# kyotovision-public/DRMNet

Measured on NVIDIA B200. Metric: refmaps rendered/sec (128^2, 2000x1000 envmap), higher is better.
Workload: dtype f32

## Files before the change

### drmnet_b200/csrc/render_tree.cu

```cuda
#include <cuda_fp16.h>
#include <math.h>
#include <string.h>

#include "common.cuh"

namespace drm {

static constexpr int TREE_THREADS = 256;
static constexpr int TREE_WARPS = 8;
static constexpr int REC4 = 5;
static constexpr int SREC4 = 7;
static constexpr int PAIR4 = 13;
static constexpr int MAX_PYR = 14;
static constexpr int STACK_CAP = 1024;
static constexpr int BUF1 = 32;
static constexpr int BUF0 = 32;
static constexpr int TREE_MAX_P = 4;
static constexpr int CHUNK = 128;
static constexpr int TREE_CHUNK = 64;

struct PyrGeom {
    int L, base;
    int H[MAX_PYR], W[MAX_PYR];
    long off[MAX_PYR];
// ... 153 lines not shown
        if (!(o > 0.f)) return;
        if (!any) { any = true; ref[0] = g0.x; ref[1] = g0.y; ref[2] = g0.z; }
        const float dx = g0.x - ref[0], dy = g0.y - ref[1], dz = g0.z - ref[2];
        om += o;
        s1[0] += o * dx; s1[1] += o * dy; s1[2] += o * dz;
        s2[0] += o * (g1.x + dx * dx); s2[1] += o * (g1.y + dy * dy); s2[2] += o * (g1.z + dz * dz);
        s2[3] += o * (g1.w + dx * dy); s2[4] += o * (g2.x + dx * dz); s2[5] += o * (g2.y + dy * dz);
        w[0] += g2.z; w[1] += g2.w; w[2] += g3.x;
        cR[0] += g3.y + g2.z * dx; cR[1] += g3.z + g2.z * dy; cR[2] += g3.w + g2.z * dz;
        cB[0] += g4.x + g3.x * dx; cB[1] += g4.y + g3.x * dy; cB[2] += g4.z + g3.x * dz;
    }
    __device__ __forceinline__ void finish(float4* r, float rh, float* mu_out) const {
        if (!any) {
            for (int i = 0; i < REC4; ++i) r[i] = make_float4(0.f, 0.f, 0.f, 0.f);
            mu_out[0] = mu_out[1] = mu_out[2] = 0.f;
            return;
        }
        const float io = 1.f / om;
        const float ax = s1[0] * io, ay = s1[1] * io, az = s1[2] * io;
        mu_out[0] = ref[0] + ax; mu_out[1] = ref[1] + ay; mu_out[2] = ref[2] + az;
        r[0] = make_float4(mu_out[0], mu_out[1], mu_out[2], rh);
        r[1] = make_float4(fmaxf(s2[0] * io - ax * ax, 0.f), fmaxf(s2[1] * io - ay * ay, 0.f), fmaxf(s2[2] * io - az * az, 0.f),
                           s2[3] * io - ax * ay);
        r[2] = make_float4(s2[4] * io - ax * az, s2[5] * io - ay * az, w[0], w[1]);
        r[3] = make_float4(w[2], cR[0] - w[0] * ax, cR[1] - w[0] * ay, cR[2] - w[0] * az);
        r[4] = make_float4(cB[0] - w[2] * ax, cB[1] - w[2] * ay, cB[2] - w[2] * az, 0.f);
    }
};

__device__ __forceinline__ float texel_f(float x) { return x; }
__device__ __forceinline__ float texel_f(__half x) { return __half2float(x); }

template <typename T>
__device__ __forceinline__ void texel_spec(const TreeArgs& g, const TreeConst& rc, const T* __restrict__ env_b, int r,
                                           int c, float* h, float& vh, float* w) {
    const float st = g.sin_t[r], ct = g.cos_t[r], sp = g.sin_p[c], cp = g.cos_p[c];
    const float dx = st * sp, dy = ct, dz = -st * cp;
    const float dom = g.domega_k * st;
    const T* e = env_b + ((size_t)r * g.We + c) * 3;
    const float sx = rc.vhat[0] + dx, sy = rc.vhat[1] + dy, sz = rc.vhat[2] + dz;
    const float len2 = fmaxf(sx * sx + sy * sy + sz * sz, 1e-12f);
    const float inv_len = rsqrtf(len2);
    vh = 0.5f * len2 * inv_len;
    h[0] = sx * inv_len; h[1] = sy * inv_len; h[2] = sz * inv_len;
    const float Fd = fresnel_dielectric_t(vh, rc.eta);
    const float mm = fminf(fmaxf(1.f - vh, 0.f), 1.f);
    const float sw = (mm * mm) * (mm * mm) * mm;
    const float a = (1.f - rc.m) * Fd + rc.m * sw, b = rc.m * (1.f - sw);
    w[0] = texel_f(e[0]) * dom * (a + b * rc.base[0]);
    w[1] = texel_f(e[1]) * dom * (a + b * rc.base[1]);
    w[2] = texel_f(e[2]) * dom * (a + b * rc.base[2]);
}

template <typename T>
__device__ __forceinline__ void texel_diff(const TreeArgs& g, const T* __restrict__ env_b, int r, int c, float* d,
                                           float* w) {
    const float st = g.sin_t[r], ct = g.cos_t[r], sp = g.sin_p[c], cp = g.cos_p[c];
    d[0] = st * sp; d[1] = ct; d[2] = -st * cp;
    const float dom = g.domega_k * st;
    const T* e = env_b + ((size_t)r * g.We + c) * 3;
    w[0] = texel_f(e[0]) * dom; w[1] = texel_f(e[1]) * dom; w[2] = texel_f(e[2]) * dom;
}

__global__ void tree_mark_used_kernel(const TreeConst* __restrict__ rc, int N, int* __restrict__ used) {
    const int k = blockIdx.x * blockDim.x + threadIdx.x;
    if (k < N && rc[k].has_diff) used[rc[k].env] = 1;
}

__global__ void env_mark_slots_kernel(const int32_t* __restrict__ ids, int n, int B, int* __restrict__ used) {
    const int i = blockIdx.x * blockDim.x + threadIdx.x;
    if (!ids) {
        if (i < B) used[i] = 1;
    } else if (i < n) {
        const int e = ids[i];
        if (e >= 0 && e < B) used[e] = 1;
    }
}

__global__ void tree_active_kernel(const TreeConst* __restrict__ rc, int n, int* __restrict__ act, int* __restrict__ nact) {
    if (blockIdx.x != 0 || threadIdx.x != 0) return;
    for (int p = 0; p <= TREE_MAX_P; ++p) {
        int c = 0;
        for (int k = 0; k < n; ++k)
            if (rc[k].pk >= p) act[p * TREE_CHUNK + c++] = k;
        nact[p] = c;
    }
}

template <bool SPEC, typename T>
__device__ __forceinline__ void pyr_from_texels(const TreeArgs& g, int lev, float4* __restrict__ pyr) {
    const PyrGeom& G = SPEC ? g.gs : g.gd;
    const int Hl = G.H[lev], Wl = G.W[lev];
    const int cell = blockIdx.x * blockDim.x + threadIdx.x;
    if (cell >= Hl * Wl) return;
    const int k = blockIdx.y;
    if (!SPEC && !g.env_used[k]) return;
    const int R = cell / Wl, C = cell - R * Wl;
    const int e = 1 << lev;
    const TreeConst* rcp = SPEC ? &g.rc[k] : nullptr;
    const T* env_b = reinterpret_cast<const T*>(g.env) + (size_t)(SPEC ? rcp->env : k) * g.He * g.We * 3;
    float4* rec = pyr + ((size_t)k * G.cells + G.off[lev] + cell) * REC4;
    if (SPEC && !rcp->has_spec) {
        for (int i = 0; i < REC4; ++i) rec[i] = make_float4(0.f, 0.f, 0.f, 0.f);
        return;
    }
    Mom M;
    M.init();
    const int r1 = min((R + 1) * e, g.He), c1 = min((C + 1) * e, g.We);
    for (int r = R * e; r < r1; ++r)
        for (int c = C * e; c < c1; ++c) {
            float x[3], w[3], vh;
            if (SPEC) texel_spec(g, *rcp, env_b, r, c, x, vh, w);
            else texel_diff(g, env_b, r, c, x, w);
            M.add_point(x, w);
        }
    float4 out[REC4];
    float mu[3];
    M.finish(out, 0.f, mu);
    float rh = 0.f;
    if (M.any) {
        for (int r = R * e; r < r1; ++r)
            for (int c = C * e; c < c1; ++c) {
                float x[3], w[3], vh;
                if (SPEC) texel_spec(g, *rcp, env_b, r, c, x, vh, w);
                else texel_diff(g, env_b, r, c, x, w);
                if (w[0] + w[1] + w[2] > 0.f) {
                    const float dx = x[0] - mu[0], dy = x[1] - mu[1], dz = x[2] - mu[2];
                    rh = fmaxf(rh, dx * dx + dy * dy + dz * dz);
                }
            }
        out[0].w = sqrtf(rh) * 1.0001f + 1e-7f;
    }
    for (int i = 0; i < REC4; ++i) rec[i] = out[i];
}

template <bool SPEC>
__global__ void pyr_from_texels_kernel(const TreeArgs g, int lev, float4* __restrict__ pyr) {
    pyr_from_texels<SPEC, float>(g, lev, pyr);
}
template <bool SPEC>
__global__ void pyr_from_texels_kernel_h(const TreeArgs g, int lev, float4* __restrict__ pyr) {
    pyr_from_texels<SPEC, __half>(g, lev, pyr);
}

__global__ void pyr_merge_kernel(PyrGeom G, int lev, float4* __restrict__ pyr, const int* __restrict__ used) {
    const int Hl = G.H[lev], Wl = G.W[lev], Hc = G.H[lev - 1], Wc = G.W[lev - 1];
    const int cell = blockIdx.x * blockDim.x + threadIdx.x;
    if (cell >= Hl * Wl) return;
    if (used && !used[blockIdx.y]) return;
    const int R = cell / Wl, C = cell - R * Wl;
    float4* base = pyr + (size_t)blockIdx.y * G.cells * REC4;
    const float4* child = base + G.off[lev - 1] * REC4;
    Mom M;
    M.init();
    for (int dr = 0; dr < 2; ++dr)
        for (int dc = 0; dc < 2; ++dc) {
            const int r = 2 * R + dr, c = 2 * C + dc;
            if (r < Hc && c < Wc) M.add_record(child + ((size_t)r * Wc + c) * REC4);
        }
    float4 out[REC4];
    float mu[3];
    M.finish(out, 0.f, mu);
    if (M.any) {
        float rh = 0.f;
        for (int dr = 0; dr < 2; ++dr)
            for (int dc = 0; dc < 2; ++dc) {
                const int r = 2 * R + dr, c = 2 * C + dc;
                if (r >= Hc || c >= Wc) continue;
                const float4* ch = child + ((size_t)r * Wc + c) * REC4;
                const float4 g0 = ch[0], g2 = ch[2], g3 = ch[3];
                if (!(g2.z + g2.w + g3.x > 0.f)) continue;
                const float dx = g0.x - mu[0], dy = g0.y - mu[1], dz = g0.z - mu[2];
                rh = fmaxf(rh, sqrtf(dx * dx + dy * dy + dz * dz) + g0.w);
            }
        out[0].w = rh * 1.0001f + 1e-7f;
    }
    float4* rec = base + (G.off[lev] + cell) * REC4;
    for (int i = 0; i < REC4; ++i) rec[i] = out[i];
}

__device__ __forceinline__ float view_term_t(const TreeConst& rc, float lz) {
    const float g1 = lz + sqrtf(lz * lz * rc.one_m_a2 + rc.alpha2);
    return lz > 0.f ? 1.f / (3.14159265358979f * rc.alpha2 * g1) : 0.f;
}

struct NodeT {
    float nx, ny, nz, nv, mult, wq, Fi;
    float q0, q1, q2, q3, q4, q5;
    float P0, P1, P2, P3, P4, P5;
    bool active;
};

__device__ __forceinline__ void make_node(const TreeArgs& g, const TreeConst& rc, int p, bool pixcov, int I, int J, bool spec,
                                          NodeT& nd) {
    const int pk = rc.pk, Sk = 1 << p, S = 1 << pk;
    const float* __restrict__ glx = g.glx[p];
// ... 92 lines not shown
}

enum : int { ACT_DROP = 0, ACT_ACCEPT = 1, ACT_REFINE = 2, ACT_HAND = 3 };

typedef float2 f2;
__device__ __forceinline__ f2 F2(float a) { return make_float2(a, a); }
__device__ __forceinline__ f2 fma2(f2 a, f2 b, f2 c) { return __ffma2_rn(a, b, c); }
__device__ __forceinline__ f2 mul2(f2 a, f2 b) { return __fmul2_rn(a, b); }
__device__ __forceinline__ f2 add2(f2 a, f2 b) { return __fadd2_rn(a, b); }
__device__ __forceinline__ f2 sub2(f2 a, f2 b) { return __fadd2_rn(a, make_float2(-b.x, -b.y)); }
__device__ __forceinline__ f2 max2(f2 a, float s) { return make_float2(fmaxf(a.x, s), fmaxf(a.y, s)); }
__device__ __forceinline__ f2 rcp2(f2 a) { return make_float2(fast_rcp(a.x), fast_rcp(a.y)); }
__device__ __forceinline__ f2 rsqrt2(f2 a) { return make_float2(fast_rsqrt(a.x), fast_rsqrt(a.y)); }
__device__ __forceinline__ f2 sqrt2(f2 a) { return make_float2(fast_sqrt(a.x), fast_sqrt(a.y)); }
__device__ __forceinline__ f2 lo(float4 v) { return make_float2(v.x, v.y); }
__device__ __forceinline__ f2 hi(float4 v) { return make_float2(v.z, v.w); }

__device__ __forceinline__ void tile_writeback(const TreeArgs& g, int p, float* red, int k, int ti, int tj, float a0, float a1,
                                               float a2, bool overwrite) {
    const int tid = threadIdx.x, lane = tid & 31, warp = tid >> 5;
    const int ln = ((warp >> 1) * 4 + (lane >> 3)) * 16 + (warp & 1) * 8 + (lane & 7);
    red[ln * 3 + 0] = a0; red[ln * 3 + 1] = a1; red[ln * 3 + 2] = a2;
    __syncthreads();
    const int Sk = 1 << p, cpt = 16 >> p;
    if (cpt < 1) return;
    const int ncell = cpt * cpt;
    for (int o = tid; o < ncell * 3; o += TREE_THREADS) {
        const int cl = o / 3, c = o - cl * 3;
        const int ci = cl / cpt, cj = cl - ci * cpt;
        const int i = ti * cpt + ci, j = tj * cpt + cj;
        if (i >= g.res || j >= g.res) continue;
        float v = 0.f;
        for (int a = 0; a < Sk; ++a)
            for (int b = 0; b < Sk; ++b) v += red[((ci * Sk + a) * 16 + cj * Sk + b) * 3 + c];
        const size_t pix = (size_t)i * g.res + j;
        const size_t idx = g.channel_first ? ((size_t)k * 3 + c) * g.res * g.res + pix : ((size_t)k * g.res * g.res + pix) * 3 + c;
        g.out[idx] = overwrite ? v : g.out[idx] + v;
    }
}

__device__ __forceinline__ void tile_of(int t, int tiles_x, int& ti, int& tj) {
    const int m = tiles_x - 1;
    if (tiles_x <= 2) { ti = t / tiles_x; tj = t - ti * tiles_x; }
    else if (t < tiles_x) { ti = 0; tj = t; }
    else if (t < 2 * tiles_x) { ti = m; tj = t - tiles_x; }
    else if (t < 2 * tiles_x + (m - 1)) { ti = 1 + t - 2 * tiles_x; tj = 0; }
    else if (t < 4 * m) { ti = 1 + t - 2 * tiles_x - (m - 1); tj = m; }
    else { const int q = t - 4 * m; ti = 1 + q / (m - 1); tj = 1 + q - (ti - 1) * (m - 1); }
}

static constexpr int SPEC_MINB[TREE_MAX_P + 1] = {3, 3, 3, 3, 3}, DIFF_MINB = 3;

static constexpr int STAT_TILE_WAIT = 50, STAT_WARP_CYCLES = 56;

struct WarpUni {
    float ax, ay, az, beta;
    float thr_p, hand_p, hz_p, xthr, rcap, kappa2;
    int limb;
};

template <int P, typename T>
__device__ __forceinline__ void tree_spec_pass(const TreeArgs g, int tid) {
    extern __shared__ __align__(16) unsigned char tree_smem[];
    const int lane = tid & 31, warp = tid >> 5;
    int* stack = reinterpret_cast<int*>(tree_smem) + warp * STACK_CAP;
    float* buf1 = reinterpret_cast<float*>(tree_smem + TREE_WARPS * STACK_CAP * 4) + warp * (BUF1 / 2 * PAIR4 * 4);
    float4* buf0 = reinterpret_cast<float4*>(tree_smem + TREE_WARPS * STACK_CAP * 4 + TREE_WARPS * (BUF1 / 2) * PAIR4 * 16) + warp * (BUF0 * 2);
    float* red = reinterpret_cast<float*>(tree_smem);

    constexpr int p = P;
    const int NG = g.res << p;
    const int tiles_x = (NG + 15) / 16;
    const int n_items = g.nact[p] * tiles_x * tiles_x;
    const bool stats = g.stats;
    long long t_warp = stats ? clock64() : 0, t_wait = 0;
    auto tile_sync = [&]() {
        const long long t = stats ? clock64() : 0;
        __syncthreads();
        if (stats) t_wait += clock64() - t;
    };
    __shared__ int next_item, next_k;
    __shared__ TreeConst rc;
    __shared__ WarpUni wu_s[TREE_WARPS];
    WarpUni& wu = wu_s[warp];
    while (true) {
    if (warp == 0) {
        int it = 0;
        if (lane == 0) it = atomicAdd(g.item_ctr, 1);
        it = __shfl_sync(0xffffffffu, it, 0);
        if (it < n_items) {
            const int kk = g.act[p * TREE_CHUNK + it % g.nact[p]];
            const int* src = reinterpret_cast<const int*>(g.rc + kk);
            int* dst = reinterpret_cast<int*>(&rc);
            for (int i = lane; i < (int)(sizeof(TreeConst) / 4); i += 32) dst[i] = src[i];
            if (lane == 0) next_k = kk;
        }
        if (lane == 0) next_item = it;
    }
    tile_sync();
    const int item = next_item;
    if (item >= n_items) break;
    const int k = next_k;
    const int tile = item / g.nact[p];
    const int pk = rc.pk;
    int ti, tj;
    tile_of(tile, tiles_x, ti, tj);
    const int I0 = ti * 16 + (warp >> 1) * 4, J0 = tj * 16 + (warp & 1) * 8;
    float a0 = 0.f, a1 = 0.f, a2 = 0.f;
    const bool pixcov = g.pixcov && p == 0 && pk > 0;

    NodeT nd;
    make_node(g, rc, p, pixcov, I0 + (lane >> 3), J0 + (lane & 7), true, nd);
    float ax, ay, az, beta;
    const bool live = rc.has_spec && warp_cone(g, p, nd, ax, ay, az, beta);
// ... 170 lines not shown
                float* s = reinterpret_cast<float*>(buf0 + (n0 >> 1) * 4) + 1;
                if (lane < 7) s[lane * 2] = lane < 3 ? (lane == 0 ? nd.nx : lane == 1 ? nd.ny : nd.nz) : 0.f;
                __syncwarp();
            }
            const int np = (n0 + 1) >> 1;
            f2 bR = F2(0.f), bG = F2(0.f), bB = F2(0.f);
#pragma unroll 2
            for (int j = 0; j < np; ++j) {
                const float4 v0 = buf0[4 * j], v1 = buf0[4 * j + 1], v2 = buf0[4 * j + 2], v3 = buf0[4 * j + 3];
                const f2 ex = sub2(NX, lo(v0)), ey = sub2(NY, hi(v0)), ez = sub2(NZ, lo(v1));
                const f2 u2 = fma2(ez, ez, fma2(ey, ey, mul2(ex, ex)));
                const f2 nh = fma2(u2, F2(-0.5f), F2(1.f));
                const f2 xc = max2(sub2(mul2(hi(v1), nh), NVp), 0.f);
                const f2 sin2 = mul2(u2, fma2(u2, F2(-0.25f), F2(1.f)));
                const f2 q = fma2(sin2, CI, F2(1.f));
                const f2 sq = sqrt2(fma2(mul2(xc, xc), OMA, A2));
                const f2 ws = mul2(xc, rcp2(mul2(mul2(q, q), add2(xc, sq))));
                bR = fma2(ws, lo(v2), bR); bG = fma2(ws, hi(v2), bG); bB = fma2(ws, lo(v3), bB);
            }
            a0 += nd.mult * (bR.x + bR.y); a1 += nd.mult * (bG.x + bG.y); a2 += nd.mult * (bB.x + bB.y);
            n0 = 0;
        };

        bool done = false;
        while (true) {
            unsigned ent = 0;
            int ntake;
            if (sp > 0) {
                ntake = min(32, sp);
                if (lane < ntake) ent = (unsigned)stack[sp - 1 - lane];
                sp -= ntake;
            } else {
                if (p > 0 && in_pos >= in_n && in_next >= 0) {
                    const int* ch = g.pool_in + (size_t)in_next * CHUNK;
                    in_next = ch[0];
                    in_n = ch[1];
                    in_list = ch + 2;
                    in_pos = 0;
                }
                if (in_pos < in_n) {
                    ntake = min(32, in_n - in_pos);
                    if (lane < ntake) ent = p == 0 ? (((unsigned)g.gs.L << 28) | (unsigned)(in_pos + lane)) : (unsigned)in_list[in_pos + lane];
                    in_pos += ntake;
                } else {
                    ntake = 0;
                    done = true;
                }
            }
            const bool has = lane < ntake;
            st_visits += ntake; st_iters += 1;
            __syncwarp();
            int act = ACT_DROP;
            const int lev = (int)(ent >> 28), id = (int)(ent & 0x0fffffffu);
            float h[3], vh = 0.f, w3[3];
            if (has) {
                float mx, my, mz, rha, wsum, vmu, im;
                if (lev > 0) {
                    const float4* rp = pyr + (g.gs.off[lev] + id) * REC4;
                    const float4 r0 = rp[0], r2 = rp[2], r3 = rp[3];
                    mx = r0.x; my = r0.y; mz = r0.z;
                    wsum = r2.z + r2.w + r3.x;
                    const float m2 = fmaxf(mx * mx + my * my + mz * mz, 1e-30f);
                    im = fast_rsqrt(m2);
                    rha = fast_radius_angle(r0.w + fmaxf(1.f - m2 * im, 0.f));
                    vmu = rc.vhat[0] * mx + rc.vhat[1] * my + rc.vhat[2] * mz;
                } else {
                    const int r = id / g.We, c = id - r * g.We;
                    texel_spec(g, rc, env_b, r, c, h, vh, w3);
                    mx = h[0]; my = h[1]; mz = h[2];
                    wsum = w3[0] + w3[1] + w3[2];
                    im = 1.f; rha = 0.f; vmu = vh;
                }
                if (wsum > 0.f) {
                    const float ax = wu.ax, ay = wu.ay, az = wu.az, beta = wu.beta;
                    const float hx = mx * im - ax, hy = my * im - ay, hz = mz * im - az;
                    const float ang = fast_chord_angle(hx * hx + hy * hy + hz * hz);
                    const float dmin = fmaxf(ang - beta - rha, 0.f);
                    const float t2 = 2.f * vmu * im * im;
                    const float adc = ax * (t2 * mx - rc.vhat[0]) + ay * (t2 * my - rc.vhat[1]) + az * (t2 * mz - rc.vhat[2]);
                    const float spread = beta + 2.f * rha + 1e-3f;
                    const float ss = __sinf(fminf(spread, 1.5607f));
                    if (spread < 1.5607f && adc <= -ss) act = ACT_DROP;
                    else if (p < pk && dmin < wu.thr_p) act = (lev == 0 || rha <= wu.hand_p * wu.thr_p) ? ACT_HAND : ACT_REFINE;
                    else if (p < pk && wu.limb && spread < 1.5607f &&
                             adc * __cosf(spread) - sqrtf(fmaxf(1.f - adc * adc, 0.f)) * ss < wu.xthr)
                        act = (lev == 0 || rha <= 0.05f) ? ACT_HAND : ACT_REFINE;
                    else if (lev > 0 && (rha > wu.rcap || rha * rha > wu.kappa2 * (rc.alpha2 + dmin * dmin) ||
                                         (2.f * rha > wu.hz_p && fabsf(adc) < ss))) act = ACT_REFINE;
                    else act = ACT_ACCEPT;
                }
            }
            {
                const unsigned mh = __ballot_sync(0xffffffffu, act == ACT_HAND);
                if (mh) {
                    const int cnt = __popc(mh);
                    if (out_cur < 0 || out_fill + cnt > CHUNK - 2) {
                        int nc = 0;
                        if (lane == 0) nc = atomicAdd(g.pool_ctr, 1);
                        nc = __shfl_sync(0xffffffffu, nc, 0);
                        if (nc >= g.pool_cap) {
                            if (lane == 0) atomicOr(g.status, 1);
                            nc = -1;
                        }
                        if (lane == 0) {
                            if (out_cur >= 0) {
                                g.pool_out[(size_t)out_cur * CHUNK] = nc;
                                g.pool_out[(size_t)out_cur * CHUNK + 1] = out_fill;
                            }
                        }
                        if (out_cur < 0) out_head = nc;
                        out_cur = nc;
                        out_fill = 0;
                    }
                    if (act == ACT_HAND && out_cur >= 0)
                        g.pool_out[(size_t)out_cur * CHUNK + 2 + out_fill + __popc(mh & ((1u << lane) - 1u))] = (int)ent;
                    if (out_cur >= 0) out_fill += cnt;
                    out_n += cnt;
                }
// ... 53 lines not shown
                        s[8] = Sxx; s[10] = Syy; s[12] = Szz; s[14] = 2.f * Sxy; s[16] = 2.f * Sxz; s[18] = 2.f * Syz;
                        s[20] = 2.f * vmu / fmaxf(1.f - trS, 1e-12f);
                        s[22] = r2.z; s[24] = r2.w; s[26] = r3.x;
                        s[28] = r3.y; s[30] = r3.z; s[32] = r3.w;
                        s[34] = r4.x; s[36] = r4.y; s[38] = r4.z;
                        s[40] = vmu; s[42] = vx * svx + vy * svy + vz * svz;
                        s[44] = svx; s[46] = svy; s[48] = svz; s[50] = 0.f;
                    } else {
                        const int slot = n0 + __popc(m0 & ((1u << lane) - 1u));
                        float* s = reinterpret_cast<float*>(buf0 + (slot >> 1) * 4) + (slot & 1);
                        s[0] = h[0]; s[2] = h[1]; s[4] = h[2]; s[6] = 2.f * vh;
                        s[8] = w3[0]; s[10] = w3[1]; s[12] = w3[2];
                    }
                }
                n1 += __popc(m1);
                n0 += __popc(m0);
                st_acc1 += __popc(m1); st_acc0 += __popc(m0);
            }
            __syncwarp();
        }
        if (p < pk && lane == 0) {
            const int nbI = (NG + 3) / 4;
            if (out_cur >= 0) {
                g.pool_out[(size_t)out_cur * CHUNK] = -1;
                g.pool_out[(size_t)out_cur * CHUNK + 1] = out_fill;
            }
            g.heads_out[(size_t)k * nbI * nbJ + (size_t)bI * nbJ + bJ] = out_head;
        }
        if (lane == 0 && g.stats) {
            atomicAdd(g.status + 16 + 4 * p, st_visits); atomicAdd(g.status + 17 + 4 * p, st_iters);
            atomicAdd(g.status + 18 + 4 * p, st_acc0); atomicAdd(g.status + 19 + 4 * p, st_acc1);
        }
        if (lane == 0) {
            if (sp_max > g.status[1]) atomicMax(g.status + 1, sp_max);
            if (out_n > g.status[2 + p]) atomicMax(g.status + 2 + p, out_n);
        }
    } else if (p < pk && lane == 0) {
        const int nbJ = (NG + 7) / 8, nbI = (NG + 3) / 4;
        const int bI = I0 >> 2, bJ = J0 >> 3;
        if (bI < nbI && bJ < nbJ) g.heads_out[(size_t)k * nbI * nbJ + (size_t)bI * nbJ + bJ] = -1;
    }
    tile_sync();
    tile_writeback(g, p, red, k, ti, tj, a0, a1, a2, false);
    tile_sync();
    }
    if (stats && lane == 0) {
        atomicAdd(g.status + STAT_TILE_WAIT + p, (int)(t_wait >> 10));
        atomicAdd(g.status + STAT_WARP_CYCLES + p, (int)((clock64() - t_warp) >> 10));
    }
}

template <int P>
__global__ void __launch_bounds__(TREE_THREADS, SPEC_MINB[P]) tree_spec_pass_kernel(const TreeArgs g) {
    tree_spec_pass<P, float>(g, threadIdx.x);
}
template <int P>
__global__ void __launch_bounds__(TREE_THREADS, SPEC_MINB[P]) tree_spec_pass_kernel_h(const TreeArgs g) {
    tree_spec_pass<P, __half>(g, threadIdx.x);
}

template <typename T>
__device__ __forceinline__ void tree_diff(const TreeArgs& g, int tid) {
    extern __shared__ __align__(16) unsigned char tree_smem[];
    const int lane = tid & 31, warp = tid >> 5;
    int* stack = reinterpret_cast<int*>(tree_smem) + warp * STACK_CAP;
    float4* buf1 = reinterpret_cast<float4*>(tree_smem + TREE_WARPS * STACK_CAP * 4) + warp * (BUF1 * SREC4);
    float* red = reinterpret_cast<float*>(tree_smem);

    const int k = blockIdx.y;
    const TreeConst rc = g.rc[k];
    const int p = g.diff_cov ? 0 : rc.pk;
    const bool pixcov = g.diff_cov && rc.pk > 0;
    const int tiles_x = ((g.res << p) + 15) / 16;
    if ((int)blockIdx.x >= tiles_x * tiles_x) return;
    const int ti = blockIdx.x / tiles_x, tj = blockIdx.x - ti * tiles_x;
    const int I0 = ti * 16 + (warp >> 1) * 4, J0 = tj * 16 + (warp & 1) * 8;
    float a0 = 0.f, a1 = 0.f, a2 = 0.f;
    NodeT nd;
    make_node(g, rc, p, pixcov, I0 + (lane >> 3), J0 + (lane & 7), false, nd);
    float ax, ay, az, beta;
    const bool live = rc.has_diff && warp_cone(g, p, nd, ax, ay, az, beta);
    if (live) {
        const float4* pyr = g.pyr_d + (size_t)rc.env * g.gd.cells * REC4;
        const T* env_b = reinterpret_cast<const T*>(g.env) + (size_t)rc.env * g.He * g.We * 3;
        const int in_n = g.gd.H[g.gd.L] * g.gd.W[g.gd.L];
        int in_pos = 0, sp = 0, n1 = 0;
        const float vx = rc.vhat[0], vy = rc.vhat[1], vz = rc.vhat[2];
        const float Fi = nd.Fi, r = rc.rough;
        const float A = 1.f - 0.5f * Fi, Bc = r * Fi, Cc = -0.5f * (1.f - 0.5f * Fi), Dc = r * (1.f - Fi), Ec = r * r * Fi;
        auto eval = [&]() {
            for (int i = 0; i < n1; ++i) {
                const float4* s = buf1 + i * SREC4;
                const float4 s0 = s[0], s1 = s[1], s2 = s[2], s3 = s[3], s4 = s[4], s5 = s[5], s6 = s[6];
                float x = nd.nx * s0.x + nd.ny * s0.y + nd.nz * s0.z;
                float nSn = nd.q0 * s1.x + nd.q1 * s1.y + nd.q2 * s1.z + nd.q3 * s2.x + nd.q4 * s2.y + nd.q5 * s2.z;
                if (pixcov)
                    nSn += s0.x * s0.x * nd.P0 + s0.y * s0.y * nd.P1 + s0.z * s0.z * nd.P2 + s0.x * s0.y * nd.P3 +
                           s0.x * s0.z * nd.P4 + s0.y * s0.z * nd.P5;
                const float w = fast_sqrt(3.f * fmaxf(nSn, 0.f));
                const bool straddle = x < w;
                const float xe = fmaxf(x + w, 0.f);
                x = straddle ? (w > 0.f ? xe * xe * fast_rcp(4.f * w) : 0.f) : x;
                x = fmaxf(x, 0.f);
                const float y = s0.w;
                const float mm = fmaxf(1.f - x, 0.f);
                const float m2 = mm * mm, m4 = m2 * m2, Fo = m4 * mm;
                const float gq = Cc + y * (Dc + Ec * y);
                const float lin = A + Bc * y + Fo * gq;
                const float gy = Dc + 2.f * Ec * y;
                const float Fo1 = -5.f * m4, Fo2 = 20.f * m2 * mm;
                const float Kx = lin + x * Fo1 * gq;
// ... 143 lines not shown
    G.cells = off > 0 ? off : 1;
}

static void gauss_legendre_t(int S, float* x, float* w) {
    for (int i = 0; i < S; ++i) {
        double z = cos(M_PI * (i + 0.75) / (S + 0.5)), pp = 1.0;
        for (int it = 0; it < 100; ++it) {
            double p1 = 1.0, p2 = 0.0;
            for (int j = 0; j < S; ++j) {
                const double p3 = p2;
                p2 = p1;
                p1 = ((2.0 * j + 1.0) * z * p2 - j * p3) / (j + 1.0);
            }
            pp = S * (z * p1 - p2) / (z * z - 1.0);
            const double dz = p1 / pp;
            z -= dz;
            if (fabs(dz) < 1e-15) break;
        }
        x[S - 1 - i] = (float)z;
        w[S - 1 - i] = (float)(1.0 / ((1.0 - z * z) * pp * pp));
    }
}

struct TreeLayout {
    PyrGeom gs, gd;
    int pk;
    size_t nblocks[TREE_MAX_P];
    int pool_cap[2];
    int* status;
    int* env_used;
    int* act;
    int* nact;
    TreeConst* rc;
    float *sin_t, *cos_t, *sin_p, *cos_p;
    float4 *pyr_s, *pyr_d;
    int* pool[2];
    int* heads[2];
};

static int log2_exact(int S) {
    for (int p = 0; p <= TREE_MAX_P; ++p)
        if ((1 << p) == S) return p;
    return -1;
}

static void make_diffuse_geom(PyrGeom& G, int He, int We) {
    int dbase = 0;
    while ((2 << dbase) * M_PI / He <= 0.03) ++dbase;
    make_geom(G, He, We, dbase);
}

static size_t tree_layout(TreeLayout& L, void* ws, int N, int B, int He, int We, int res, int S, bool prepared = false) {
    make_geom(L.gs, He, We, 1);
    make_diffuse_geom(L.gd, He, We);
    L.pk = S > 0 ? log2_exact(S) : TREE_MAX_P;
    const int NC = N < TREE_CHUNK ? N : TREE_CHUNK;
    Carver c(ws);
    L.status = c.take<int>(64);
    L.rc = c.take<TreeConst>(N);
    L.env_used = prepared ? nullptr : c.take<int>(B);
    L.act = c.take<int>((TREE_MAX_P + 1) * TREE_CHUNK);
    L.nact = c.take<int>(16);
    L.sin_t = c.take<float>(He);
    L.cos_t = c.take<float>(He);
    L.sin_p = c.take<float>(We);
    L.cos_p = c.take<float>(We);
    L.pyr_s = c.take<float4>((size_t)NC * L.gs.cells * REC4);
    L.pyr_d = prepared ? nullptr : c.take<float4>((size_t)B * L.gd.cells * REC4);
    size_t need[2] = {1, 1}, needh[2] = {1, 1};
    for (int p = 0; p < L.pk; ++p) {
        const size_t NG = (size_t)res << p;
        L.nblocks[p] = ((NG + 3) / 4) * ((NG + 7) / 8);
        static const size_t budget[TREE_MAX_P] = {64, 24, 10, 6};
        const size_t per_block = budget[p];
        const size_t n = (size_t)NC * L.nblocks[p] * per_block + 64;
        if (n > need[p & 1]) need[p & 1] = n;
        if ((size_t)NC * L.nblocks[p] > needh[p & 1]) needh[p & 1] = (size_t)NC * L.nblocks[p];
    }
    for (int i = 0; i < 2; ++i) {
        L.pool_cap[i] = (int)(need[i] < 0x7fffffff / CHUNK ? need[i] : 0x7fffffff / CHUNK);
        L.pool[i] = c.take<int>((size_t)L.pool_cap[i] * CHUNK);
        L.heads[i] = c.take<int>(needh[i]);
    }
    return c.used();
}

struct EnvPyrLayout {
    PyrGeom gd;
    float4* pyr;
    float *sin_t, *cos_t, *sin_p, *cos_p;
    int* used;
};

static size_t env_pyr_layout(EnvPyrLayout& L, void* buf, int B, int He, int We) {
    make_diffuse_geom(L.gd, He, We);
    Carver c(buf);
    L.pyr = c.take<float4>((size_t)B * L.gd.cells * REC4);
    L.sin_t = c.take<float>(He);
    L.cos_t = c.take<float>(He);
    L.sin_p = c.take<float>(We);
    L.cos_p = c.take<float>(We);
    L.used = c.take<int>(B);
    return c.used();
}

static bool env_sizes_ok(int B, int He, int We) {
    return B > 0 && B <= 65535 && He > 0 && We > 0 && (long)He * We < (1L << 28);
}

static constexpr size_t TREE_SMEM = (size_t)TREE_WARPS * STACK_CAP * 4 + (size_t)TREE_WARPS * (BUF1 / 2) * PAIR4 * 16 +
                                    (size_t)TREE_WARPS * BUF0 * 2 * 16;
static_assert(BUF1 * SREC4 <= (BUF1 / 2) * PAIR4 + 8 * BUF0, "the diffuse pass stages its records in the same region");

static constexpr int MAX_DEVICES = 64;

template <typename T> struct TexelKernels;
template <> struct TexelKernels<float> {
    template <int P> static constexpr void (*spec)(TreeArgs) = tree_spec_pass_kernel<P>;
    static constexpr void (*diff)(TreeArgs) = tree_diff_kernel;
    template <bool SPEC> static constexpr void (*pyr)(TreeArgs, int, float4*) = pyr_from_texels_kernel<SPEC>;
};
template <> struct TexelKernels<__half> {
    template <int P> static constexpr void (*spec)(TreeArgs) = tree_spec_pass_kernel_h<P>;
    static constexpr void (*diff)(TreeArgs) = tree_diff_kernel_h;
    template <bool SPEC> static constexpr void (*pyr)(TreeArgs, int, float4*) = pyr_from_texels_kernel_h<SPEC>;
};

template <typename T>
static int launch_diffuse_pyramids(const TreeArgs& g, int B, float4* pyr, cudaStream_t st) {
    if (g.gd.L < 1) return 0;
    const int tb = 128;
    const int first = g.gd.base > 0 ? g.gd.base : 1;
    const int nb = g.gd.H[first] * g.gd.W[first];
    int launches = 0;
    TexelKernels<T>::template pyr<false><<<dim3((nb + tb - 1) / tb, B), tb, 0, st>>>(g, first, pyr);
    ++launches;
    for (int l = first + 1; l <= g.gd.L; ++l) {
        const int nl = g.gd.H[l] * g.gd.W[l];
        pyr_merge_kernel<<<dim3((nl + tb - 1) / tb, B), tb, 0, st>>>(g.gd, l, pyr, g.env_used);
        ++launches;
    }
    return launches;
}

template <int P, typename T>
static cudaError_t launch_spec_pass(const TreeArgs& a, long items, cudaStream_t st) {
    static int resident[MAX_DEVICES];
    void (*kernel)(TreeArgs) = TexelKernels<T>::template spec<P>;
    cudaError_t e = cudaFuncSetAttribute(kernel, cudaFuncAttributeMaxDynamicSharedMemorySize, (int)TREE_SMEM);
    if (e == cudaSuccess)
        e = cudaFuncSetAttribute(kernel, cudaFuncAttributePreferredSharedMemoryCarveout, cudaSharedmemCarveoutMaxShared);
    int dev = 0;
    if (e == cudaSuccess) e = cudaGetDevice(&dev);
    if (e != cudaSuccess) return e;
    int per_sm = 0, sms = 0;
    int* slot = dev < MAX_DEVICES ? &resident[dev] : &per_sm;
    if (*slot == 0) {
        e = cudaOccupancyMaxActiveBlocksPerMultiprocessor(&per_sm, kernel, TREE_THREADS, TREE_SMEM);
        if (e == cudaSuccess) e = cudaDeviceGetAttribute(&sms, cudaDevAttrMultiProcessorCount, dev);
        if (e != cudaSuccess) return e;
        *slot = max(per_sm, 1) * sms;
    }
    const int grid = (int)(items < *slot ? items : *slot);
    kernel<<<grid, TREE_THREADS, TREE_SMEM, st>>>(a);
    return cudaGetLastError();
}

}

using namespace drm;

extern "C" size_t drm_render_workspace_bytes(int N, int B, int He, int We, int res, int S) {
    if (N <= 0 || B <= 0 || He <= 0 || We <= 0 || res <= 0 || (S != 0 && log2_exact(S) < 0)) return 0;
    if ((long)He * We >= (1L << 28)) return 0;
    TreeLayout L;
    return tree_layout(L, nullptr, N, B, He, We, res, S);
}

extern "C" size_t drm_render_prepared_workspace_bytes(int N, int B, int He, int We, int res, int S) {
    if (N <= 0 || B <= 0 || He <= 0 || We <= 0 || res <= 0 || (S != 0 && log2_exact(S) < 0)) return 0;
    if ((long)He * We >= (1L << 28)) return 0;
    TreeLayout L;
    return tree_layout(L, nullptr, N, B, He, We, res, S, true);
}

extern "C" size_t drm_env_pyramid_bytes(int B, int He, int We) {
    if (!env_sizes_ok(B, He, We)) return 0;
    EnvPyrLayout P;
    return env_pyr_layout(P, nullptr, B, He, We);
}

template <typename T>
static int env_pyramid_build(const T* env, int B, int He, int We, const int32_t* ids, int n_ids, void* pyramids,
                             size_t pyramid_bytes, cudaStream_t st) {
    EnvPyrLayout P;
    const size_t need = env_pyr_layout(P, pyramids, B, He, We);
    DRM_REQUIRE(pyramid_bytes >= need, "env_pyramid_build: pyramid buffer of %zu bytes needed for B=%d He=%d We=%d, %zu given",
                need, B, He, We, pyramid_bytes);
    if (ids && n_ids == 0) return DRM_OK;
    TreeArgs g;
    memset(&g, 0, sizeof(g));
// ... 28 lines not shown
    DRM_CHECK_CUDA(cudaMemcpyAsync(status_host, workspace, 40 * sizeof(int), cudaMemcpyDeviceToHost,
                                   static_cast<cudaStream_t>(cuda_stream)));
    return DRM_OK;
}

template <typename T>
static int render_refmaps(const T* env, int B, int He, int We, const int32_t* env_index, const float* z6,
                          const float* view3, const uint8_t* flip, int N, int res, int S, float alpha_min,
                          int channel_first, float* out, void* workspace, size_t workspace_bytes, void* cuda_stream,
                          const DrmRenderOptions* opts, bool prepared = false, const void* pyramids = nullptr,
                          size_t pyramid_bytes = 0) {
    DRM_REQUIRE(env && z6 && view3 && out, "render: null pointer");
    DRM_REQUIRE(!prepared || pyramids, "render: null pointer (pyramids)");
    DRM_REQUIRE(N > 0 && B > 0 && He > 0 && We > 0 && res > 0, "render: N=%d B=%d He=%d We=%d res=%d must be positive", N, B, He, We, res);
    DRM_REQUIRE(S == 0 || log2_exact(S) >= 0, "render: footprint_S=%d must be 0 (per render) or 1, 2, 4, 8, 16", S);
    DRM_REQUIRE(res <= 4096, "render: res=%d too large", res);
    DRM_REQUIRE(B <= 65535, "render: at most 65535 envmaps per call (B=%d)", B);
    DRM_REQUIRE((long)He * We < (1L << 28), "render: envmap of %d x %d texels is too large", He, We);
    if (prepared) {
        EnvPyrLayout P;
        const size_t pneed = env_pyr_layout(P, nullptr, B, He, We);
        DRM_REQUIRE(pyramid_bytes >= pneed, "render: pyramid buffer of %zu bytes needed for B=%d He=%d We=%d, %zu given",
                    pneed, B, He, We, pyramid_bytes);
    }
    cudaStream_t st = static_cast<cudaStream_t>(cuda_stream);
    DrmRenderOptions o;
    drm_render_default_options(&o);
    if (opts) o = *opts;
    const int32_t* S_per_render = o.footprint_per_render;
    const int S_layout = S_per_render ? 0 : S;
    TreeLayout L;
    const size_t need = tree_layout(L, workspace, N, B, He, We, res, S_layout, prepared);
    if (prepared) L.pyr_d = static_cast<float4*>(const_cast<void*>(pyramids));
    if (!workspace || workspace_bytes < need) {
        set_error("render: workspace of %zu bytes needed, %zu given", need, workspace_bytes);
        return DRM_EWORKSPACE;
    }
    if (!(alpha_min > 0.f)) alpha_min = fmaxf(1e-3f, (float)(1.25 * M_PI / He));

    TreeArgs g;
    memset(&g, 0, sizeof(g));
    g.env = reinterpret_cast<const float*>(env); g.sin_t = L.sin_t; g.cos_t = L.cos_t; g.sin_p = L.sin_p; g.cos_p = L.cos_p;
    g.pyr_s = L.pyr_s; g.pyr_d = L.pyr_d; g.status = L.status; g.env_used = L.env_used; g.act = L.act; g.nact = L.nact;
    g.gs = L.gs; g.gd = L.gd;
    g.B = B; g.He = He; g.We = We; g.res = res; g.pk = L.pk; g.channel_first = channel_first;
    g.cell = (float)(M_PI / res);
    g.domega_k = (float)((2.0 * M_PI / We) * (M_PI / He));
    g.kappa = o.kappa; g.rcap = o.rcap; g.rcap_simple = o.rcap_simple; g.hz = o.horizon; g.hz_in = fmaxf(o.horizon, o.horizon_inner * fminf(1.f, powf((float)(M_PI / 128.0) / g.cell, 0.25f))); g.hz_nv = o.horizon_inner_nv; g.hz_fin = fmaxf(o.horizon, o.horizon_finest * fminf(1.f, powf((float)(M_PI / 128.0) / g.cell, 0.25f))); g.kappa_d = o.kappa_diffuse; g.hz_d = o.horizon_diffuse; g.hand = o.hand_over; g.limb_nv = o.limb_nv; g.limb_boost = o.limb_boost; g.limb_x = o.limb_x; g.limb_hand = o.limb_hand; g.limb_ramp = o.limb_ramp; g.limb_sub = o.limb_sub; g.limb_cells = o.limb_cells;
    for (int p = 0; p <= TREE_MAX_P; ++p) gauss_legendre_t(1 << p, g.glx[p], g.glw[p]);
    g.diff_cov = (o.pixel_covariance && g.cell <= 0.03f) ? 1 : 0;
    g.stats = o.collect_stats;

    const int tb = 128;
    DRM_CHECK_CUDA(cudaMemsetAsync(L.status, 0, 64 * sizeof(int), st));
    tree_tables_kernel<<<(max(He, We) + tb - 1) / tb, tb, 0, st>>>(L.sin_t, L.cos_t, L.sin_p, L.cos_p, He, We);
    const float grow = (float)fmin(10.0, pow(fmax(1.0, (M_PI / res) / (M_PI / 128.0)), 1.5));
    tree_setup_kernel<<<(N + tb - 1) / tb, tb, 0, st>>>(z6, view3, flip, env_index, N, B, alpha_min, g.cell,
                                                       o.level_scale * grow, (o.pixel_covariance ? o.level_scale0 : o.level_scale) * grow,
                                                       o.full_second_order ? o.alpha_full2 : 1e30f, o.pixel_covariance, o.flat_scale,
                                                       S, S_per_render, L.rc, L.status);
    count_launches(2);
    if (!prepared) {
        DRM_CHECK_CUDA(cudaMemsetAsync(L.env_used, 0, sizeof(int) * B, st));
        tree_mark_used_kernel<<<(N + tb - 1) / tb, tb, 0, st>>>(L.rc, N, L.env_used);
        count_launches(1 + launch_diffuse_pyramids<T>(g, B, L.pyr_d, st));
    }
    DRM_CHECK_CUDA(cudaFuncSetAttribute(TexelKernels<T>::diff, cudaFuncAttributeMaxDynamicSharedMemorySize, (int)TREE_SMEM));
    DRM_CHECK_CUDA(cudaFuncSetAttribute(TexelKernels<T>::diff, cudaFuncAttributePreferredSharedMemoryCarveout, cudaSharedmemCarveoutMaxShared));
    const size_t per_render_out = (size_t)res * res * 3;
    for (int k0 = 0; k0 < N; k0 += TREE_CHUNK) {
        const int n = N - k0 < TREE_CHUNK ? N - k0 : TREE_CHUNK;
        TreeArgs a = g;
        a.rc = L.rc + k0;
        a.N = n;
        a.out = out + (size_t)k0 * per_render_out;
        tree_active_kernel<<<1, 32, 0, st>>>(a.rc, n, L.act, L.nact);
        count_launches(1);
        if (L.gs.L >= 1) {
            const int n1 = L.gs.H[1] * L.gs.W[1];
            TexelKernels<T>::template pyr<true><<<dim3((n1 + tb - 1) / tb, n), tb, 0, st>>>(a, 1, L.pyr_s);
            count_launches(1);
            for (int l = 2; l <= L.gs.L; ++l) {
                const int nl = L.gs.H[l] * L.gs.W[l];
                pyr_merge_kernel<<<dim3((nl + tb - 1) / tb, n), tb, 0, st>>>(L.gs, l, L.pyr_s, nullptr);
                count_launches(1);
            }
        }
        {
            const int pd = a.diff_cov ? 0 : L.pk;
            const int NGd = res << pd;
            const int tiles = ((NGd + 15) / 16) * ((NGd + 15) / 16);
            TexelKernels<T>::diff<<<dim3(tiles, n), TREE_THREADS, TREE_SMEM, st>>>(a);
            count_launches(1);
        }
        for (int p = 0; p <= L.pk; ++p) {
            a.pixcov = (o.pixel_covariance && p == 0) ? 1 : 0;
            a.pool_in = nullptr; a.heads_in = nullptr; a.pool_out = nullptr; a.heads_out = nullptr; a.pool_ctr = nullptr;
            if (p > 0) { a.pool_in = L.pool[(p - 1) & 1]; a.heads_in = L.heads[(p - 1) & 1]; }
            if (p < L.pk) {
                a.pool_out = L.pool[p & 1]; a.heads_out = L.heads[p & 1]; a.pool_cap = L.pool_cap[p & 1];
                a.pool_ctr = L.status + 8 + p;
                DRM_CHECK_CUDA(cudaMemsetAsync(a.pool_ctr, 0, sizeof(int), st));
            }
            const int NG = res << p;
            const long items = (long)((NG + 15) / 16) * ((NG + 15) / 16) * n;
            a.item_ctr = L.status + 44 + p;
            DRM_CHECK_CUDA(cudaMemsetAsync(a.item_ctr, 0, sizeof(int), st));
            switch (p) {
                case 0: DRM_CHECK_CUDA((launch_spec_pass<0, T>(a, items, st))); break;
                case 1: DRM_CHECK_CUDA((launch_spec_pass<1, T>(a, items, st))); break;
                case 2: DRM_CHECK_CUDA((launch_spec_pass<2, T>(a, items, st))); break;
                case 3: DRM_CHECK_CUDA((launch_spec_pass<3, T>(a, items, st))); break;
                default: DRM_CHECK_CUDA((launch_spec_pass<4, T>(a, items, st))); break;
            }
            count_launches(1);
        }
    }
    DRM_CHECK_CUDA(cudaGetLastError());
    return DRM_OK;
}

extern "C" int drm_render_refmaps_opts(const float* env, int B, int He, int We, const int32_t* env_index, const float* z6,
                                       const float* view3, const uint8_t* flip, int N, int res, int S, float alpha_min,
                                       int channel_first, float* out, void* workspace, size_t workspace_bytes,
                                       void* cuda_stream, const DrmRenderOptions* opts) {
    return render_refmaps(env, B, He, We, env_index, z6, view3, flip, N, res, S, alpha_min, channel_first, out, workspace,
                          workspace_bytes, cuda_stream, opts);
}

extern "C" int drm_render_refmaps_half(const void* env, int B, int He, int We, const int32_t* env_index, const float* z6,
                                       const float* view3, const uint8_t* flip, int N, int res, int S, float alpha_min,
                                       int channel_first, float* out, void* workspace, size_t workspace_bytes,
                                       void* cuda_stream, const DrmRenderOptions* opts) {
    return render_refmaps(static_cast<const __half*>(env), B, He, We, env_index, z6, view3, flip, N, res, S, alpha_min,
                          channel_first, out, workspace, workspace_bytes, cuda_stream, opts);
}

extern "C" int drm_render_refmaps_prepared(const void* env, int env_half, const void* pyramids, size_t pyramid_bytes,
                                           int B, int He, int We, const int32_t* env_index, const float* z6,
                                           const float* view3, const uint8_t* flip, int N, int res, int S,
                                           float alpha_min, int channel_first, float* out, void* workspace,
                                           size_t workspace_bytes, void* cuda_stream, const DrmRenderOptions* opts) {
    if (env_half)
        return render_refmaps(static_cast<const __half*>(env), B, He, We, env_index, z6, view3, flip, N, res, S,
                              alpha_min, channel_first, out, workspace, workspace_bytes, cuda_stream, opts, true,
                              pyramids, pyramid_bytes);
    return render_refmaps(static_cast<const float*>(env), B, He, We, env_index, z6, view3, flip, N, res, S, alpha_min,
                          channel_first, out, workspace, workspace_bytes, cuda_stream, opts, true, pyramids,
                          pyramid_bytes);
}

extern "C" int drm_render_refmaps(const float* env, int B, int He, int We, const int32_t* env_index, const float* z6,
                                  const float* view3, const uint8_t* flip, int N, int res, int S, float alpha_min,
                                  int channel_first, float* out, void* workspace, size_t workspace_bytes,
                                  void* cuda_stream) {
    return drm_render_refmaps_opts(env, B, He, We, env_index, z6, view3, flip, N, res, S, alpha_min, channel_first, out,
                                   workspace, workspace_bytes, cuda_stream, nullptr);
}

extern "C" void drm_render_default_options(DrmRenderOptions* o) {
    if (!o) return;
    o->kappa = 0.1f;
    o->rcap = 0.06f;
    o->rcap_simple = 0.035f;
    o->horizon = 0.03f;
    o->kappa_diffuse = 0.1f;
// ... 22 lines not shown
```

Baseline: 380.2.

## Precompute per-texel specular records in pyramid build and read them in tree traversal

Adds a kernel that evaluates the per-render specular texel terms (half vector, Fresnel-weighted radiance) once for every 2x2 quad. It stores them in a quad-interleaved texel buffer appended to the pyramid and builds the level-1 records from them directly. The specular tree passes now load these precomputed float4 pairs at leaf level instead of recomputing trig, Fresnel and env lookups on every revisit. The cost is extra workspace memory and global traffic to write all texels per render, and the spec pass is now always the float path. Optional stats counters for leaf visits are also added.

```diff
diff --git a/drmnet_b200/csrc/render_tree.cu b/drmnet_b200/csrc/render_tree.cu
--- a/drmnet_b200/csrc/render_tree.cu
+++ b/drmnet_b200/csrc/render_tree.cu
@@ -229,6 +229,10 @@
     w[2] = texel_f(e[2]) * dom * (a + b * rc.base[2]);
 }
 
+__device__ __forceinline__ int tex_index(int r, int c, int W1) {
+    return (((r >> 1) * W1 + (c >> 1)) << 2) | ((r & 1) << 1) | (c & 1);
+}
+
 template <typename T>
 __device__ __forceinline__ void texel_diff(const TreeArgs& g, const T* __restrict__ env_b, int r, int c, float* d,
                                            float* w) {
@@ -311,6 +315,54 @@
     for (int i = 0; i < REC4; ++i) rec[i] = out[i];
 }
 
+template <typename T>
+__device__ __forceinline__ void pyr_spec_records(const TreeArgs& g, float4* __restrict__ pyr) {
+    const int H1 = (g.He + 1) >> 1, W1 = (g.We + 1) >> 1;
+    const int cell = blockIdx.x * blockDim.x + threadIdx.x;
+    if (cell >= H1 * W1) return;
+    const int k = blockIdx.y;
+    const TreeConst& rc = g.rc[k];
+    float4* rec = g.gs.L >= 1 ? pyr + ((size_t)k * g.gs.cells + g.gs.off[1] + cell) * REC4 : nullptr;
+    if (!rc.has_spec) {
+        if (rec)
+            for (int i = 0; i < REC4; ++i) rec[i] = make_float4(0.f, 0.f, 0.f, 0.f);
+        return;
+    }
+    const int R = cell / W1, C = cell - R * W1;
+    const T* env_b = reinterpret_cast<const T*>(g.env) + (size_t)rc.env * g.He * g.We * 3;
+    float4* tex = pyr + ((size_t)k * g.gs.cells + g.gs.off[0]) * REC4 + (size_t)cell * 8;
+    float x[4][3], w[4][3];
+    bool in[4];
+    Mom M;
+    M.init();
+#pragma unroll
+    for (int q = 0; q < 4; ++q) {
+        const int r = 2 * R + (q >> 1), c = 2 * C + (q & 1);
+        in[q] = r < g.He && c < g.We;
+        if (!in[q]) continue;
+        float vh;
+        texel_spec(g, rc, env_b, r, c, x[q], vh, w[q]);
+        tex[2 * q] = make_float4(x[q][0], x[q][1], x[q][2], 2.f * vh);
+        tex[2 * q + 1] = make_float4(w[q][0], w[q][1], w[q][2], w[q][0] + w[q][1] + w[q][2]);
+        M.add_point(x[q], w[q]);
+    }
+    if (!rec) return;
+    float4 out[REC4];
+    float mu[3];
+    M.finish(out, 0.f, mu);
+    if (M.any) {
+        float rh = 0.f;
+#pragma unroll
+        for (int q = 0; q < 4; ++q)
+            if (in[q] && w[q][0] + w[q][1] + w[q][2] > 0.f) {
+                const float dx = x[q][0] - mu[0], dy = x[q][1] - mu[1], dz = x[q][2] - mu[2];
+                rh = fmaxf(rh, dx * dx + dy * dy + dz * dz);
+            }
+        out[0].w = sqrtf(rh) * 1.0001f + 1e-7f;
+    }
+    for (int i = 0; i < REC4; ++i) rec[i] = out[i];
+}
+
 template <bool SPEC>
 __global__ void pyr_from_texels_kernel(const TreeArgs g, int lev, float4* __restrict__ pyr) {
     pyr_from_texels<SPEC, float>(g, lev, pyr);
@@ -319,6 +371,8 @@
 __global__ void pyr_from_texels_kernel_h(const TreeArgs g, int lev, float4* __restrict__ pyr) {
     pyr_from_texels<SPEC, __half>(g, lev, pyr);
 }
+__global__ void pyr_spec_records_kernel(const TreeArgs g, float4* __restrict__ pyr) { pyr_spec_records<float>(g, pyr); }
+__global__ void pyr_spec_records_kernel_h(const TreeArgs g, float4* __restrict__ pyr) { pyr_spec_records<__half>(g, pyr); }
 
 __global__ void pyr_merge_kernel(PyrGeom G, int lev, float4* __restrict__ pyr, const int* __restrict__ used) {
     const int Hl = G.H[lev], Wl = G.W[lev], Hc = G.H[lev - 1], Wc = G.W[lev - 1];
@@ -517,6 +571,7 @@
 static constexpr int SPEC_MINB[TREE_MAX_P + 1] = {3, 3, 3, 3, 3}, DIFF_MINB = 3;
 
 static constexpr int STAT_TILE_WAIT = 50, STAT_WARP_CYCLES = 56;
+static constexpr int STAT_LEV0_VISITS = 36, STAT_LEV0_ITERS = 64, STATUS_WORDS = 72;
 
 struct WarpUni {
     float ax, ay, az, beta;
@@ -524,7 +579,7 @@
     int limb;
 };
 
-template <int P, typename T>
+template <int P, typename T, bool REC>
 __device__ __forceinline__ void tree_spec_pass(const TreeArgs g, int tid) {
     extern __shared__ __align__(16) unsigned char tree_smem[];
     const int lane = tid & 31, warp = tid >> 5;
@@ -801,6 +856,13 @@
             __syncwarp();
             int act = ACT_DROP;
             const int lev = (int)(ent >> 28), id = (int)(ent & 0x0fffffffu);
+            if (REC && stats) {
+                const unsigned m0v = __ballot_sync(0xffffffffu, has && lev == 0);
+                if (m0v && lane == 0) {
+                    atomicAdd(g.status + STAT_LEV0_VISITS + p, __popc(m0v));
+                    atomicAdd(g.status + STAT_LEV0_ITERS + p, 1);
+                }
+            }
             float h[3], vh = 0.f, w3[3];
             if (has) {
                 float mx, my, mz, rha, wsum, vmu, im;
@@ -813,6 +875,15 @@
                     im = fast_rsqrt(m2);
                     rha = fast_radius_angle(r0.w + fmaxf(1.f - m2 * im, 0.f));
                     vmu = rc.vhat[0] * mx + rc.vhat[1] * my + rc.vhat[2] * mz;
+                } else if constexpr (REC) {
+                    const int r = id / g.We, c = id - r * g.We;
+                    const float4* tp = pyr + g.gs.off[0] * REC4 + (size_t)tex_index(r, c, (g.We + 1) >> 1) * 2;
+                    const float4 t0 = tp[0], t1 = tp[1];
+                    h[0] = t0.x; h[1] = t0.y; h[2] = t0.z; vh = 0.5f * t0.w;
+                    w3[0] = t1.x; w3[1] = t1.y; w3[2] = t1.z;
+                    mx = h[0]; my = h[1]; mz = h[2];
+                    wsum = t1.w;
+                    im = 1.f; rha = 0.f; vmu = vh;
                 } else {
                     const int r = id / g.We, c = id - r * g.We;
                     texel_spec(g, rc, env_b, r, c, h, vh, w3);
@@ -972,11 +1043,15 @@
 
 template <int P>
 __global__ void __launch_bounds__(TREE_THREADS, SPEC_MINB[P]) tree_spec_pass_kernel(const TreeArgs g) {
-    tree_spec_pass<P, float>(g, threadIdx.x);
+    tree_spec_pass<P, float, false>(g, threadIdx.x);
 }
 template <int P>
 __global__ void __launch_bounds__(TREE_THREADS, SPEC_MINB[P]) tree_spec_pass_kernel_h(const TreeArgs g) {
-    tree_spec_pass<P, __half>(g, threadIdx.x);
+    tree_spec_pass<P, __half, false>(g, threadIdx.x);
+}
+template <int P>
+__global__ void __launch_bounds__(TREE_THREADS, SPEC_MINB[P]) tree_spec_pass_rec_kernel(const TreeArgs g) {
+    tree_spec_pass<P, float, true>(g, threadIdx.x);
 }
 
 template <typename T>
@@ -1226,11 +1301,17 @@
 
 static size_t tree_layout(TreeLayout& L, void* ws, int N, int B, int He, int We, int res, int S, bool prepared = false) {
     make_geom(L.gs, He, We, 1);
+    {
+        const long levels = L.gs.L >= 1 ? L.gs.cells : 0;
+        L.gs.off[0] = (levels + 7) / 8 * 8;
+        const long tex4 = (long)((He + 1) / 2) * ((We + 1) / 2) * 8;
+        L.gs.cells = (L.gs.off[0] + (tex4 + REC4 - 1) / REC4 + 7) / 8 * 8;
+    }
     make_diffuse_geom(L.gd, He, We);
     L.pk = S > 0 ? log2_exact(S) : TREE_MAX_P;
     const int NC = N < TREE_CHUNK ? N : TREE_CHUNK;
     Carver c(ws);
-    L.status = c.take<int>(64);
+    L.status = c.take<int>(STATUS_WORDS);
     L.rc = c.take<TreeConst>(N);
     L.env_used = prepared ? nullptr : c.take<int>(B);
     L.act = c.take<int>((TREE_MAX_P + 1) * TREE_CHUNK);
@@ -1290,15 +1371,28 @@
 
 template <typename T> struct TexelKernels;
 template <> struct TexelKernels<float> {
-    template <int P> static constexpr void (*spec)(TreeArgs) = tree_spec_pass_kernel<P>;
     static constexpr void (*diff)(TreeArgs) = tree_diff_kernel;
     template <bool SPEC> static constexpr void (*pyr)(TreeArgs, int, float4*) = pyr_from_texels_kernel<SPEC>;
+    static constexpr void (*records)(TreeArgs, float4*) = pyr_spec_records_kernel;
 };
 template <> struct TexelKernels<__half> {
-    template <int P> static constexpr void (*spec)(TreeArgs) = tree_spec_pass_kernel_h<P>;
     static constexpr void (*diff)(TreeArgs) = tree_diff_kernel_h;
     template <bool SPEC> static constexpr void (*pyr)(TreeArgs, int, float4*) = pyr_from_texels_kernel_h<SPEC>;
+    static constexpr void (*records)(TreeArgs, float4*) = pyr_spec_records_kernel_h;
 };
+
+template __global__ void tree_spec_pass_kernel<0>(const TreeArgs);
+template __global__ void tree_spec_pass_kernel<1>(const TreeArgs);
+template __global__ void tree_spec_pass_kernel<2>(const TreeArgs);
+template __global__ void tree_spec_pass_kernel<3>(const TreeArgs);
+template __global__ void tree_spec_pass_kernel<4>(const TreeArgs);
+template __global__ void tree_spec_pass_kernel_h<0>(const TreeArgs);
+template __global__ void tree_spec_pass_kernel_h<1>(const TreeArgs);
+template __global__ void tree_spec_pass_kernel_h<2>(const TreeArgs);
+template __global__ void tree_spec_pass_kernel_h<3>(const TreeArgs);
+template __global__ void tree_spec_pass_kernel_h<4>(const TreeArgs);
+template __global__ void pyr_from_texels_kernel<true>(const TreeArgs, int, float4*);
+template __global__ void pyr_from_texels_kernel_h<true>(const TreeArgs, int, float4*);
 
 template <typename T>
 static int launch_diffuse_pyramids(const TreeArgs& g, int B, float4* pyr, cudaStream_t st) {
@@ -1317,10 +1411,10 @@
     return launches;
 }
 
-template <int P, typename T>
+template <int P>
 static cudaError_t launch_spec_pass(const TreeArgs& a, long items, cudaStream_t st) {
     static int resident[MAX_DEVICES];
-    void (*kernel)(TreeArgs) = TexelKernels<T>::template spec<P>;
+    void (*kernel)(TreeArgs) = tree_spec_pass_rec_kernel<P>;
     cudaError_t e = cudaFuncSetAttribute(kernel, cudaFuncAttributeMaxDynamicSharedMemorySize, (int)TREE_SMEM);
     if (e == cudaSuccess)
         e = cudaFuncSetAttribute(kernel, cudaFuncAttributePreferredSharedMemoryCarveout, cudaSharedmemCarveoutMaxShared);
@@ -1455,7 +1549,7 @@
     g.stats = o.collect_stats;
 
     const int tb = 128;
-    DRM_CHECK_CUDA(cudaMemsetAsync(L.status, 0, 64 * sizeof(int), st));
+    DRM_CHECK_CUDA(cudaMemsetAsync(L.status, 0, STATUS_WORDS * sizeof(int), st));
     tree_tables_kernel<<<(max(He, We) + tb - 1) / tb, tb, 0, st>>>(L.sin_t, L.cos_t, L.sin_p, L.cos_p, He, We);
     const float grow = (float)fmin(10.0, pow(fmax(1.0, (M_PI / res) / (M_PI / 128.0)), 1.5));
     tree_setup_kernel<<<(N + tb - 1) / tb, tb, 0, st>>>(z6, view3, flip, env_index, N, B, alpha_min, g.cell,
@@ -1479,9 +1573,9 @@
         a.out = out + (size_t)k0 * per_render_out;
         tree_active_kernel<<<1, 32, 0, st>>>(a.rc, n, L.act, L.nact);
         count_launches(1);
-        if (L.gs.L >= 1) {
-            const int n1 = L.gs.H[1] * L.gs.W[1];
-            TexelKernels<T>::template pyr<true><<<dim3((n1 + tb - 1) / tb, n), tb, 0, st>>>(a, 1, L.pyr_s);
+        {
+            const int n1 = ((He + 1) / 2) * ((We + 1) / 2);
+            TexelKernels<T>::records<<<dim3((n1 + tb - 1) / tb, n), tb, 0, st>>>(a, L.pyr_s);
             count_launches(1);
             for (int l = 2; l <= L.gs.L; ++l) {
                 const int nl = L.gs.H[l] * L.gs.W[l];
@@ -1510,11 +1604,11 @@
             a.item_ctr = L.status + 44 + p;
             DRM_CHECK_CUDA(cudaMemsetAsync(a.item_ctr, 0, sizeof(int), st));
             switch (p) {
-                case 0: DRM_CHECK_CUDA((launch_spec_pass<0, T>(a, items, st))); break;
-                case 1: DRM_CHECK_CUDA((launch_spec_pass<1, T>(a, items, st))); break;
-                case 2: DRM_CHECK_CUDA((launch_spec_pass<2, T>(a, items, st))); break;
-                case 3: DRM_CHECK_CUDA((launch_spec_pass<3, T>(a, items, st))); break;
-                default: DRM_CHECK_CUDA((launch_spec_pass<4, T>(a, items, st))); break;
+                case 0: DRM_CHECK_CUDA((launch_spec_pass<0>(a, items, st))); break;
+                case 1: DRM_CHECK_CUDA((launch_spec_pass<1>(a, items, st))); break;
+                case 2: DRM_CHECK_CUDA((launch_spec_pass<2>(a, items, st))); break;
+                case 3: DRM_CHECK_CUDA((launch_spec_pass<3>(a, items, st))); break;
+                default: DRM_CHECK_CUDA((launch_spec_pass<4>(a, items, st))); break;
             }
             count_launches(1);
         }
```

After: 383.6 (median of 6 runs). Within noise of the previous version (+0.9%).
